# google/fedjax

Hardware: AMD Instinct MI355X
Metric: device-resident aggregated client-delta GB/s, K clients × P fp32 params (higher is better)
Workload: dtype f32; 1 GPU; configs[2]: mean aggregator, 1024 clients x 4 M-param (4,194,304) fp32 deltas; clients=1024, params=4194304, clients_per_gpu=1024, parallelism=client-sharded x1, buckets=1, nontemporal=True, variant=0, fused_l2_norms=False, fused_server_step=none

## Files before the change

fedjax_amd/csrc/fjhost.cpp:

```cpp

#include <Python.h>
#include <structmember.h>

#include <ATen/ATen.h>
#include <c10/hip/HIPFunctions.h>
#include <c10/hip/HIPStream.h>
#include <torch/csrc/autograd/python_variable.h>

#include <algorithm>
#include <chrono>
#include <cmath>
#include <cstdlib>
#include <cstdint>
#include <cstring>
#include <deque>
#include <functional>
#include <unordered_map>
#include <vector>

#include "fjagg.h"
#include "fjtree.h"

namespace {

// ... 2476 lines not shown
    std::vector<int64_t> pp(L, 0), st(3 * L, 0);
    PyObject* side[4] = {params, mt, vt, mo};
    for (int i = 0; i < 4; ++i) {
      if (side[i] == Py_None) {
        if (i == 0) Py_RETURN_NONE;
        continue;
      }
      w.out = i == 0 ? pp.data() : st.data() + (i - 1) * L;
      w.leaf = 0;
      const int r = walk(spec, side[i], w);
      if (r < 0) return nullptr;
      if (r > 0 || w.leaf != static_cast<size_t>(L)) Py_RETURN_NONE;
    }
    std::vector<int64_t> ptrs(static_cast<size_t>(K * L));
    for (int64_t l = 0; l < L; ++l) ptrs[l] = reinterpret_cast<int64_t>(row0[l].data_ptr());
    for (Py_ssize_t k = 1; k < K; ++k) {
      w.out = ptrs.data() + k * L;
      w.leaf = 0;
      const int r = walk(spec, trees[k], w);
      if (r < 0) return nullptr;
      if (r > 0 || w.leaf != static_cast<size_t>(L)) Py_RETURN_NONE;
    }
    std::vector<uint8_t> elem(L, 0);
    bool any_elem = false;
    for (int64_t l = 0; l < L; ++l) {
      int64_t bits = pp[l] | st[l] | st[L + l] | st[2 * L + l];
      for (Py_ssize_t k = 0; k < K; ++k) bits |= ptrs[k * L + l];
      elem[l] = (bits & 15) != 0;
      any_elem = any_elem || elem[l];
    }
    auto plan = reinterpret_cast<PlanFn>(plan_addr);
    const uint8_t* mask = any_elem ? elem.data() : nullptr;
    const int64_t nblk = plan(kF32, 0, leaf_n.data(), mask, static_cast<int>(L), nullptr, 0);
    if (nblk < 1) Py_RETURN_NONE;
    const int64_t nw = (K + 1) / 2, n = K * L + 2 * L + 2 * nblk + nw + 3 * L;
    if (upload_refused_in_capture(reinterpret_cast<unsigned long long>(
                                      c10::hip::getCurrentHIPStream(static_cast<c10::DeviceIndex>(dev)).stream()),
                                  "the server step's pytree fold"))
      return nullptr;
    at::Tensor img = at::empty({n}, at::TensorOptions().dtype(at::kLong).pinned_memory(true));
    int64_t* p = img.data_ptr<int64_t>();
    std::memcpy(p, ptrs.data(), sizeof(int64_t) * K * L);
    std::memcpy(p + K * L, pp.data(), sizeof(int64_t) * L);
    std::memcpy(p + K * L + L, leaf_n.data(), sizeof(int64_t) * L);
    if (plan(kF32, 0, leaf_n.data(), mask, static_cast<int>(L), p + K * L + 2 * L, nblk) != nblk) Py_RETURN_NONE;
    int64_t* wp = p + K * L + 2 * L + 2 * nblk;
    wp[nw - 1] = 0;
    std::memcpy(wp, wf.data(), 4 * K);
    std::memcpy(wp + nw, st.data(), sizeof(int64_t) * 3 * L);
    at::Tensor dimg = img.to(at::Device(at::kCUDA, static_cast<c10::DeviceIndex>(dev)), true);
    const int64_t* dp = dimg.data_ptr<int64_t>();
    const double job_bytes = 4.0 * static_cast<double>(total) * static_cast<double>(K);
    const int flags = job_bytes >= nt_min ? kNontemporal : 0;
    const float scale = static_cast<float>(W > 0.0 ? 1.0 / W : 0.0);
    const unsigned long long stream =
        reinterpret_cast<unsigned long long>(c10::hip::getCurrentHIPStream(static_cast<c10::DeviceIndex>(dev)).stream());
    const int rc = reinterpret_cast<UpdFn>(upd_addr)(kF32, dp, static_cast<int>(L), K, nblk,
                                                      reinterpret_cast<const float*>(dp + K * L + 2 * L + 2 * nblk),
                                                      scale, reinterpret_cast<const void*>(desc_addr),
                                                      dp + K * L + 2 * L + 2 * nblk + nw, flags,
                                                      reinterpret_cast<void*>(stream));
    return PyLong_FromLong(rc);
  } catch (const std::exception& e) {
    PyErr_SetString(PyExc_RuntimeError, e.what());
    return nullptr;
  }
}


struct WTObject {
  PyObject_HEAD
  PyObject* tree;
  PyObject* weight;
  PyObject* cap;
  PyObject* value;
};

struct ChainObject {
  PyObject_HEAD
  PyObject* tip;
  PyObject* buf;
  PyObject* budget;
  PyObject* views;
};

struct PSObject {
  PyObject_HEAD
  PyObject* root;
  PyObject* parent;
  PyObject* cap;
  PyObject* weight;
  PyObject* value;
  PyObject* chain;
  PyObject* ticket;
  PyObject* ref;
  PyObject* bcap;
  long long n, bytes, idx, tok;
  PyObject* weakreflist;
};

#define FJ_OBJ_MEMBER(T, f) {const_cast<char*>("_" #f), T_OBJECT, offsetof(T, f), 0, nullptr}
#define FJ_LL_MEMBER(T, f) {const_cast<char*>("_" #f), T_LONGLONG, offsetof(T, f), 0, nullptr}

PyMemberDef kWTMembers[] = {FJ_OBJ_MEMBER(WTObject, tree), FJ_OBJ_MEMBER(WTObject, weight),
                            FJ_OBJ_MEMBER(WTObject, cap), FJ_OBJ_MEMBER(WTObject, value), {nullptr}};
PyMemberDef kChainMembers[] = {{const_cast<char*>("tip"), T_OBJECT, offsetof(ChainObject, tip), 0, nullptr},
                               {const_cast<char*>("buf"), T_OBJECT, offsetof(ChainObject, buf), 0, nullptr},
                               {const_cast<char*>("budget"), T_OBJECT, offsetof(ChainObject, budget), 0, nullptr},
                               {const_cast<char*>("views"), T_OBJECT, offsetof(ChainObject, views), 0, nullptr},
                               {nullptr}};
PyMemberDef kPSMembers[] = {FJ_OBJ_MEMBER(PSObject, root),   FJ_OBJ_MEMBER(PSObject, parent),
                            FJ_OBJ_MEMBER(PSObject, cap),    FJ_OBJ_MEMBER(PSObject, weight),
                            FJ_OBJ_MEMBER(PSObject, value),  FJ_OBJ_MEMBER(PSObject, chain),
                            FJ_OBJ_MEMBER(PSObject, ticket), FJ_OBJ_MEMBER(PSObject, ref),
                            FJ_OBJ_MEMBER(PSObject, bcap),   FJ_LL_MEMBER(PSObject, n),
                            FJ_LL_MEMBER(PSObject, bytes),   FJ_LL_MEMBER(PSObject, idx),
                            FJ_LL_MEMBER(PSObject, tok),
                            {const_cast<char*>("__weaklistoffset__"), T_PYSSIZET, offsetof(PSObject, weakreflist),
                             READONLY, nullptr},
                            {nullptr}};

int wt_traverse(PyObject* o, visitproc visit, void* arg) {
  auto* x = reinterpret_cast<WTObject*>(o);
  Py_VISIT(Py_TYPE(o));
  Py_VISIT(x->tree);
  Py_VISIT(x->weight);
  Py_VISIT(x->cap);
  Py_VISIT(x->value);
  return 0;
}
int wt_clear(PyObject* o) {
  auto* x = reinterpret_cast<WTObject*>(o);
  Py_CLEAR(x->tree);
  Py_CLEAR(x->weight);
  Py_CLEAR(x->cap);
  Py_CLEAR(x->value);
  return 0;
}
void wt_dealloc(PyObject* o) {
  PyTypeObject* tp = Py_TYPE(o);
  PyObject_GC_UnTrack(o);
  wt_clear(o);
  tp->tp_free(o);
  Py_DECREF(tp);
}

int chain_traverse(PyObject* o, visitproc visit, void* arg) {
  auto* x = reinterpret_cast<ChainObject*>(o);
  Py_VISIT(Py_TYPE(o));
  Py_VISIT(x->tip);
  Py_VISIT(x->buf);
  Py_VISIT(x->budget);
  Py_VISIT(x->views);
  return 0;
}
int chain_clear(PyObject* o) {
  auto* x = reinterpret_cast<ChainObject*>(o);
  Py_CLEAR(x->tip);
  Py_CLEAR(x->buf);
  Py_CLEAR(x->budget);
  Py_CLEAR(x->views);
  return 0;
}
void chain_dealloc(PyObject* o) {
  PyTypeObject* tp = Py_TYPE(o);
  PyObject_GC_UnTrack(o);
  chain_clear(o);
  tp->tp_free(o);
  Py_DECREF(tp);
}

int ps_traverse(PyObject* o, visitproc visit, void* arg) {
  auto* x = reinterpret_cast<PSObject*>(o);
  Py_VISIT(Py_TYPE(o));
  Py_VISIT(x->root);
  Py_VISIT(x->parent);
  Py_VISIT(x->cap);
  Py_VISIT(x->weight);
  Py_VISIT(x->value);
  Py_VISIT(x->chain);
  Py_VISIT(x->ticket);
  Py_VISIT(x->ref);
  Py_VISIT(x->bcap);
  return 0;
}
int ps_clear(PyObject* o) {
  auto* x = reinterpret_cast<PSObject*>(o);
  Py_CLEAR(x->root);
  Py_CLEAR(x->parent);
  Py_CLEAR(x->cap);
  Py_CLEAR(x->weight);
  Py_CLEAR(x->value);
  Py_CLEAR(x->chain);
  Py_CLEAR(x->ticket);
  Py_CLEAR(x->ref);
  Py_CLEAR(x->bcap);
  return 0;
}
void ps_dealloc(PyObject* o) {
  PyTypeObject* tp = Py_TYPE(o);
  PyObject_GC_UnTrack(o);
  if (reinterpret_cast<PSObject*>(o)->weakreflist) PyObject_ClearWeakRefs(o);
  ps_clear(o);
  tp->tp_free(o);
  Py_DECREF(tp);
}

PyType_Slot kWTSlots[] = {{Py_tp_dealloc, reinterpret_cast<void*>(wt_dealloc)},
                          {Py_tp_traverse, reinterpret_cast<void*>(wt_traverse)},
                          {Py_tp_clear, reinterpret_cast<void*>(wt_clear)},
                          {Py_tp_members, kWTMembers},
                          {Py_tp_new, reinterpret_cast<void*>(PyType_GenericNew)},
                          {Py_tp_doc, const_cast<char*>("fields of tree_util.WeightedTree")},
                          {0, nullptr}};
PyType_Slot kChainSlots[] = {{Py_tp_dealloc, reinterpret_cast<void*>(chain_dealloc)},
                             {Py_tp_traverse, reinterpret_cast<void*>(chain_traverse)},
                             {Py_tp_clear, reinterpret_cast<void*>(chain_clear)},
                             {Py_tp_members, kChainMembers},
                             {Py_tp_new, reinterpret_cast<void*>(PyType_GenericNew)},
                             {Py_tp_doc, const_cast<char*>("fields of tree_util._Chain")},
                             {0, nullptr}};
PyType_Slot kPSSlots[] = {{Py_tp_dealloc, reinterpret_cast<void*>(ps_dealloc)},
                          {Py_tp_traverse, reinterpret_cast<void*>(ps_traverse)},
                          {Py_tp_clear, reinterpret_cast<void*>(ps_clear)},
                          {Py_tp_members, kPSMembers},
                          {Py_tp_new, reinterpret_cast<void*>(PyType_GenericNew)},
                          {Py_tp_doc, const_cast<char*>("fields of tree_util.PendingSum")},
                          {0, nullptr}};
constexpr unsigned kBaseFlags = Py_TPFLAGS_DEFAULT | Py_TPFLAGS_BASETYPE | Py_TPFLAGS_HAVE_GC;
PyType_Spec kWTSpec = {"_fjhost.WeightedBase", sizeof(WTObject), 0, kBaseFlags, kWTSlots};
PyType_Spec kChainSpec = {"_fjhost.ChainBase", sizeof(ChainObject), 0, kBaseFlags, kChainSlots};
PyType_Spec kPSSpec = {"_fjhost.PendingBase", sizeof(PSObject), 0, kBaseFlags, kPSSlots};

struct FastState {
  PyTypeObject* ticket = nullptr;
  PyTypeObject* norm_view = nullptr;
  PyObject* py_l2[2] = {nullptr, nullptr};
  PyObject* py_fold_ticket = nullptr;
  PyTypeObject* wt = nullptr;
  PyTypeObject* ps = nullptr;
  PyTypeObject* chain = nullptr;
  PyObject* py_tree_weight = nullptr;
  PyObject* py_tree_add = nullptr;
  bool defer = true;
  long long max_clients = 4095, flush_bytes = 256LL << 20, flush_clients = 64;
  PyObject* last = nullptr;
  PyObject* pool_buf = nullptr;
  PyObject* pool_views = nullptr;
  PyObject* pool_all = nullptr;
  std::vector<std::pair<PyObject*, PyObject*>> retired;
  std::vector<unsigned long long> retired_stream;
  unsigned long long pool_stream = 0;
  PyObject* d_view_ticket = nullptr;
  PyObject* d_ticket_node = nullptr;
  long long pool_want = 0;
  double refill_us = 0.0;
  long long pool_reuses = 0, pool_builds = 0;
};
FastState g_fast;

PyObject* fast_install(PyObject*, PyObject* args) {
  PyObject *wt, *ps, *ch, *ftw, *fta;
  if (!PyArg_ParseTuple(args, "O!O!O!OO", &PyType_Type, &wt, &PyType_Type, &ps, &PyType_Type, &ch, &ftw, &fta))
    return nullptr;
  if (!PyCallable_Check(ftw) || !PyCallable_Check(fta)) {
    PyErr_SetString(PyExc_TypeError, "fast_install: fallbacks must be callable");
    return nullptr;
  }
  Py_INCREF(wt), Py_INCREF(ps), Py_INCREF(ch), Py_INCREF(ftw), Py_INCREF(fta);
  Py_XSETREF(g_fast.wt, reinterpret_cast<PyTypeObject*>(wt));
  Py_XSETREF(g_fast.ps, reinterpret_cast<PyTypeObject*>(ps));
  Py_XSETREF(g_fast.chain, reinterpret_cast<PyTypeObject*>(ch));
  Py_XSETREF(g_fast.py_tree_weight, ftw);
  Py_XSETREF(g_fast.py_tree_add, fta);
  Py_RETURN_NONE;
}

PyObject* fast_config(PyObject*, PyObject* args) {
  int en;
  long long mc, fb, fc;
  if (!PyArg_ParseTuple(args, "pLLL", &en, &mc, &fb, &fc)) return nullptr;
  g_fast.defer = en != 0;
  g_fast.max_clients = mc;
  g_fast.flush_bytes = fb;
  g_fast.flush_clients = fc;
  Py_RETURN_NONE;
}

PyObject* set_last(PyObject*, PyObject* node) {
  PyObject* wr = PyWeakref_NewRef(node, nullptr);
  if (!wr) return nullptr;
  Py_XSETREF(g_fast.last, wr);
  Py_RETURN_NONE;
}
PyObject* last(PyObject*, PyObject*) {
  PyObject* o = g_fast.last ? PyWeakref_GetObject(g_fast.last) : Py_None;
  Py_INCREF(o);
  return o;
}

inline int deferrable_weight(PyObject* w) {
  if (PyFloat_CheckExact(w)) return 1;
  if (!PyLong_CheckExact(w)) return 0;
  int of = 0;
  const long long v = PyLong_AsLongLongAndOverflow(w, &of);
  if (v == -1 && PyErr_Occurred()) return -1;
  return (!of && v > -(1LL << 53) && v < (1LL << 53)) ? 1 : 0;
}

PyObject* fast_tree_weight(PyObject*, PyObject* const* args, Py_ssize_t nargs, PyObject* kwnames) {
  if (!g_fast.wt || !g_fast.py_tree_weight) {
    PyErr_SetString(PyExc_RuntimeError, "fedjax_amd.tree_util is not installed (fast_install)");
    return nullptr;
  }
  if (nargs == 2 && kwnames == nullptr) {
    const int ok = deferrable_weight(args[1]);
    if (ok < 0) return nullptr;
    if (ok) {
      PyObject* cap = capture_impl(args[0], -1);
      if (!cap) return nullptr;
      if (cap != Py_None) {
        auto* o = reinterpret_cast<WTObject*>(g_fast.wt->tp_alloc(g_fast.wt, 0));
        if (!o) {
          Py_DECREF(cap);
          return nullptr;
        }
        Py_INCREF(args[0]);
        o->tree = args[0];
        Py_INCREF(args[1]);
        o->weight = args[1];
        o->cap = cap;
        return reinterpret_cast<PyObject*>(o);
      }
      Py_DECREF(cap);
    }
  }
  return PyObject_Vectorcall(g_fast.py_tree_weight, args, nargs, kwnames);
}

inline bool flush_due(const PSObject* p) { return p->bytes >= g_fast.flush_bytes && p->n >= g_fast.flush_clients; }

PyObject* fast_tree_add(PyObject*, PyObject* const* args, Py_ssize_t nargs, PyObject* kwnames) {
  if (!g_fast.ps || !g_fast.py_tree_add) {
    PyErr_SetString(PyExc_RuntimeError, "fedjax_amd.tree_util is not installed (fast_install)");
    return nullptr;
  }
  if (nargs == 2 && kwnames == nullptr && g_fast.defer && Py_TYPE(args[1]) == g_fast.wt &&
      Py_TYPE(args[0]) == g_fast.ps) {
    auto* r = reinterpret_cast<WTObject*>(args[1]);
    auto* p = reinterpret_cast<PSObject*>(args[0]);
    auto* ch = reinterpret_cast<ChainObject*>(p->chain);
    if (r->tree && r->tree != Py_None && r->cap && PyTuple_CheckExact(r->cap) && PyTuple_GET_SIZE(r->cap) >= 4 &&
        (!p->value || p->value == Py_None) && p->tok >= 0 && ch && Py_TYPE(ch) == g_fast.chain &&
        ch->tip == args[0] && ch->budget && PyLong_CheckExact(ch->budget)) {
      const long long tok = PyLong_AsLongLong(PyTuple_GET_ITEM(r->cap, 3));
      const long long nb = PyLong_AsLongLong(PyTuple_GET_ITEM(r->cap, 2));
      const long long budget = PyLong_AsLongLong(ch->budget);
      if (PyErr_Occurred()) return nullptr;
      if (tok == p->tok && p->n + 1 <= g_fast.max_clients && p->bytes + nb <= budget && !flush_due(p)) {
        auto* q = reinterpret_cast<PSObject*>(g_fast.ps->tp_alloc(g_fast.ps, 0));
        if (!q) return nullptr;
        Py_INCREF(p);
        q->parent = args[0];
        Py_INCREF(r->cap);
        q->cap = r->cap;
        Py_INCREF(r->weight);
        q->weight = r->weight;
        Py_INCREF(ch);
        q->chain = reinterpret_cast<PyObject*>(ch);
        Py_XINCREF(p->ref);
        q->ref = p->ref;
        q->n = p->n + 1;
        q->bytes = p->bytes + nb;
        q->idx = p->idx + 1;
        q->tok = p->tok;
        Py_INCREF(q);
        Py_XSETREF(ch->tip, reinterpret_cast<PyObject*>(q));
        PyObject* wr = PyWeakref_NewRef(reinterpret_cast<PyObject*>(q), nullptr);
        if (!wr) {
          Py_DECREF(q);
          return nullptr;
        }
        Py_XSETREF(g_fast.last, wr);
        return reinterpret_cast<PyObject*>(q);
      }
    }
  }
  return PyObject_Vectorcall(g_fast.py_tree_add, args, nargs, kwnames);
}


PyObject* fast_install_norms(PyObject*, PyObject* args) {
  PyObject *tk, *nv, *f0, *f1, *ft = Py_None;
  if (!PyArg_ParseTuple(args, "O!O!OO|O", &PyType_Type, &tk, &PyType_Type, &nv, &f0, &f1, &ft)) return nullptr;
  Py_INCREF(tk), Py_INCREF(nv), Py_INCREF(f0), Py_INCREF(f1), Py_INCREF(ft);
  Py_XSETREF(g_fast.ticket, reinterpret_cast<PyTypeObject*>(tk));
  Py_XSETREF(g_fast.norm_view, reinterpret_cast<PyTypeObject*>(nv));
  Py_XSETREF(g_fast.py_l2[0], f0);
  Py_XSETREF(g_fast.py_l2[1], f1);
  Py_XSETREF(g_fast.py_fold_ticket, ft);
  PyObject* dv = PyObject_GetAttrString(nv, "_ticket");
  PyObject* dn = dv ? PyObject_GetAttrString(tk, "node") : nullptr;
  if (!dv || !dn || !Py_TYPE(dv)->tp_descr_set || !Py_TYPE(dn)->tp_descr_set || !Py_TYPE(dv)->tp_descr_get) {
    Py_XDECREF(dv), Py_XDECREF(dn);
    PyErr_Clear();
    PyErr_SetString(PyExc_TypeError, "fast_install_norms: _NormView._ticket and _Ticket.node must be __slots__");
    return nullptr;
  }
  Py_XSETREF(g_fast.d_view_ticket, dv);
  Py_XSETREF(g_fast.d_ticket_node, dn);
  Py_RETURN_NONE;
}

inline int slot_set(PyObject* descr, PyObject* obj, PyObject* v) { return Py_TYPE(descr)->tp_descr_set(descr, obj, v); }

PyObject* solo_stale_error() {
  PyErr_SetString(PyExc_RuntimeError,
                  "a client delta passed to tree_l2_norm / tree_l2_squared was modified (a leaf updated in place) "
                  "before its lazy norm was computed; the reference takes the norm of the value at that call. Add "
                  "copies, or call fedjax_amd.tree_util.set_lazy_norms(False)");
  return nullptr;
}

PyObject* solo_config(PyObject*, PyObject* args) {
  int on;
  long long mp, bb;
  unsigned long long rf, wf, pf;
  PyObject* pb;
  if (!PyArg_ParseTuple(args, "pLLKKKO", &on, &mp, &bb, &rf, &wf, &pf, &pb)) return nullptr;
  g_solo.on = on != 0;
  g_solo.max_pending = std::max<long long>(1, std::min<long long>(mp, 1LL << 20));
  g_solo.budget = std::max<long long>(0, bb);
  if (rf) g_solo.rows_fn = rf;
  if (wf) g_solo.l2ws_fn = wf;
  if (pf) g_solo.plan_fn = pf;
  if (pb != Py_None) {
    Py_INCREF(pb);
    Py_XSETREF(g_solo.py_budget, pb);
  }
  Py_RETURN_NONE;
}

// ... 747 lines not shown
    links.push_back(p);
    if (!p->parent || p->parent == Py_None) {
      base = p->root;
      break;
    }
    if (Py_TYPE(p->parent) != g_fast.ps) Py_RETURN_NONE;
    p = reinterpret_cast<PSObject*>(p->parent);
  }
  if (links.empty() || !base) Py_RETURN_NONE;
  std::reverse(links.begin(), links.end());
  PyObject* bcap = links[0]->bcap;
  if (!bcap || bcap == Py_None) Py_RETURN_NONE;
  const Py_ssize_t K = static_cast<Py_ssize_t>(links.size()) + 1;
  thread_local std::vector<PyObject*> caps, weights;
  caps.resize(K);
  weights.resize(K);
  static PyObject* one = PyLong_FromLong(1);
  caps[0] = bcap;
  weights[0] = one;
  for (Py_ssize_t j = 1; j < K; ++j) {
    caps[j] = links[j - 1]->cap;
    weights[j] = links[j - 1]->weight;
    if (!caps[j] || !weights[j]) Py_RETURN_NONE;
  }
  static PyObject* node_name = PyUnicode_InternFromString("node");
  thread_local std::vector<size_t> waiting;
  waiting.clear();
  for (size_t j = 0; j < links.size(); ++j) {
    PyObject* tk = links[j]->ticket;
    if (!tk || tk == Py_None) continue;
    PyObject* tn = (Py_TYPE(tk) == g_fast.ticket && g_fast.d_ticket_node)
                       ? Py_TYPE(g_fast.d_ticket_node)->tp_descr_get(g_fast.d_ticket_node, tk, nullptr)
                       : PyObject_GetAttr(tk, node_name);
    if (!tn) return nullptr;
    const bool w = tn != Py_None;
    Py_DECREF(tn);
    if (w) waiting.push_back(j);
  }
  try {
    L2Rows rows{};
    bool use_rows = false;
    c10::DeviceIndex rows_dev = -1;
    if (!waiting.empty() && rows_addr) {
      PyObject* ch0 = links[0]->chain;
      bool one = ch0 && Py_TYPE(ch0) == g_fast.chain;
      for (size_t j = 1; one && j < links.size(); ++j)
        one = links[j]->chain == ch0 && links[j]->idx == links[0]->idx + static_cast<long long>(j);
      PyObject* buf = one ? reinterpret_cast<ChainObject*>(ch0)->buf : nullptr;
      if (buf && THPVariable_Check(buf)) {
        const at::Tensor& b = THPVariable_Unpack(buf);
        const int64_t i0 = links[0]->idx, n = static_cast<int64_t>(links.size());
        PyObject* bt0 = PyTuple_Check(bcap) && PyTuple_GET_SIZE(bcap) > 0 ? PyTuple_GET_ITEM(bcap, 0) : nullptr;
        const int fold_dev = bt0 && PyTuple_Check(bt0) && PyTuple_GET_SIZE(bt0) > 0 &&
                                     THPVariable_Check(PyTuple_GET_ITEM(bt0, 0))
                                 ? THPVariable_Unpack(PyTuple_GET_ITEM(bt0, 0)).get_device()
                                 : -2;
        if (b.dim() == 2 && b.size(0) == 2 && b.is_contiguous() && b.scalar_type() == at::kFloat && b.is_cuda() &&
            b.get_device() == fold_dev && i0 >= 0 && i0 + n <= b.size(1)) {
          float* row0 = b.data_ptr<float>() + i0;
          rows = L2Rows{reinterpret_cast<WsumL2RowsFn>(rows_addr), row0, row0 + b.size(1), 1};
          use_rows = true;
          rows_dev = b.get_device();
        }
      }
    }
    at::Tensor l2;
    PyObject* l2obj = Py_None;
    if (!waiting.empty() && !use_rows) {
      PyObject* t0 = PyTuple_Check(bcap) && PyTuple_GET_SIZE(bcap) > 0 ? PyTuple_GET_ITEM(bcap, 0) : nullptr;
      if (!t0 || !PyTuple_Check(t0) || PyTuple_GET_SIZE(t0) < 1 || !THPVariable_Check(PyTuple_GET_ITEM(t0, 0)))
        Py_RETURN_NONE;
      l2 = at::empty({K}, THPVariable_Unpack(PyTuple_GET_ITEM(t0, 0)).options().dtype(at::kFloat));
      l2obj = THPVariable_Wrap(l2);
      if (!l2obj) return nullptr;
    }
    Py_INCREF(base);
    PyObject* got = fold_caps_impl(base, caps.data(), weights.data(), K, scale, has_scale != 0, nt_min, plan_addr,
                                   wsum_addr, l2_addr, l2ws_addr, l2obj, use_rows ? &rows : nullptr);
    if (got && PyTuple_Check(got)) {
      const double now = now_s();
      const auto* tip = reinterpret_cast<PSObject*>(node);
      const double bytes = static_cast<double>(tip->bytes) * (1.0 + 1.0 / std::max<long long>(1, tip->n));
      g_mean.busy_until = std::max(now, g_mean.busy_until) + bytes / g_mean.peak;
    }
    Py_DECREF(base);
    if (l2obj != Py_None) Py_DECREF(l2obj);
    if (!got || waiting.empty() || !PyTuple_Check(got) || PyLong_AsLong(PyTuple_GET_ITEM(got, 0)) != 0) return got;
    typedef int (*FillFn)(const float*, float*, float*, int64_t, void*);
    auto fill = reinterpret_cast<FillFn>(fill_addr);
    for (size_t j = use_rows ? links.size() : 0; j < links.size();) {
      PyObject* ch = links[j]->chain;
      const size_t j0 = j;
      while (j < links.size() && links[j]->chain == ch &&
             links[j]->idx == links[j0]->idx + static_cast<long long>(j - j0))
        ++j;
      PyObject* buf = ch && Py_TYPE(ch) == g_fast.chain ? reinterpret_cast<ChainObject*>(ch)->buf : nullptr;
      if (buf && THPVariable_Check(buf)) {
        const at::Tensor& b = THPVariable_Unpack(buf);
        const int64_t i0 = links[j0]->idx, n = std::min<int64_t>(static_cast<int64_t>(j - j0), b.size(1) - i0);
        if (n <= 0) continue;
        if (fill && b.is_contiguous() && b.scalar_type() == at::kFloat && b.is_cuda() &&
            b.get_device() == l2.get_device()) {
          float* row0 = b.data_ptr<float>() + i0;
          const hipStream_t s = c10::hip::getCurrentHIPStream(l2.get_device()).stream();
          const int rc = fill(l2.data_ptr<float>() + 1 + j0, row0, row0 + b.size(1), n, s);
          if (rc != 0) {
            Py_DECREF(got);
            PyErr_Format(PyExc_RuntimeError, "fjtree_norms_fill failed (%d)", rc);
            return nullptr;
          }
          continue;
        }
        const at::Tensor src = l2.narrow(0, 1 + static_cast<int64_t>(j0), n);
        b.select(0, 0).narrow(0, i0, n).copy_(src);
        at::Tensor dst = b.select(0, 1).narrow(0, i0, n);
        at::sqrt_out(dst, src);
      }
    }
    for (size_t j : waiting) {
      PyObject* tk = links[j]->ticket;
      if ((Py_TYPE(tk) == g_fast.ticket && g_fast.d_ticket_node ? slot_set(g_fast.d_ticket_node, tk, Py_None)
                                                                 : PyObject_SetAttr(tk, node_name, Py_None)) != 0) {
        Py_DECREF(got);
        return nullptr;
      }
      Py_CLEAR(links[j]->ticket);
    }
    if (has_scale) {
      auto* ch = reinterpret_cast<ChainObject*>(links.back()->chain);
      if (ch && Py_TYPE(ch) == g_fast.chain && ch->tip == node) {
        Py_CLEAR(ch->buf);
        Py_CLEAR(ch->views);
      }
      if (refill_pool(use_rows ? rows_dev : l2.get_device()) != 0) {
        Py_DECREF(got);
        return nullptr;
      }
    }
    return got;
  } catch (const std::exception& e) {
    PyErr_SetString(PyExc_RuntimeError, e.what());
    return nullptr;
  }
}

PyObject* image_paths(PyObject*, PyObject*) {
  return Py_BuildValue("{s:L,s:L}", "kernel_args", g_image_karg, "uploaded", g_image_upload);
}

PyObject* host_timers(PyObject*, PyObject*) {
  static const char* names[kTPhases] = {"spec",  "checks", "outputs", "plan",           "image",
                                        "upload", "launch", "wrap",    "first_launch_at"};
  PyObject* d = PyDict_New();
  if (!d) return nullptr;
  for (int i = 0; i < kTPhases; ++i) {
    PyObject* v = PyFloat_FromDouble(g_timer_calls ? g_timers[i] / g_timer_calls : 0.0);
    PyDict_SetItemString(d, names[i], v);
    Py_DECREF(v);
    g_timers[i] = 0.0;
  }
  PyObject* c = PyLong_FromLongLong(g_timer_calls);
  PyDict_SetItemString(d, "calls", c);
  Py_DECREF(c);
  g_timer_calls = 0;
  return d;
}

PyMethodDef kMethods[] = {
    {"host_timers", host_timers, METH_NOARGS, "mean per-call microseconds of fold_table's phases (resets)"},
    {"image_paths", image_paths, METH_NOARGS, "fold_table launches with the image in kernel arguments / uploaded"},
    {"gather_rows", gather_rows, METH_VARARGS, "pointer table of K client pytrees (see fjhost.cpp)"},
    {"leaf_versions", leaf_versions, METH_VARARGS, "torch in-place version counters of K pytrees' leaves"},
    {"fold_weights", fold_weights, METH_VARARGS, "f32/i32 weights and W of Python-number weights"},
    {"capture", capture, METH_VARARGS, "leaves + version sum of a tree for a lazy tree_weight"},
    {"capture_probe", capture_probe, METH_VARARGS, "ns per call of capture's parts (profiling)"},
    {"solo_probe", solo_probe, METH_VARARGS, "ns per call of the lazy norm capture's parts (profiling)"},
    {"matches", matches, METH_VARARGS, "tree holds exactly the captured leaves, unmodified"},
    {"compatible", compatible, METH_VARARGS, "tree_add(a, b) is the fast case (structure, float32 leaves)"},
    {"append_check", append_check, METH_VARARGS, "deferred tree_add: structure + capture check in one walk"},
    {"norm_view", norm_view, METH_VARARGS, "0-d view of buf[row, index] as a tensor subclass"},
    {"table_from_caps", table_from_caps, METH_VARARGS, "pointer table of captured leaves, version check"},
    {"fold_caps", fold_caps, METH_VARARGS, "a deferred running sum's fold from its captures, one call"},
    {"leaf_fold", leaf_fold, METH_VARARGS, "fjtree_fold_leaves over 1-2 operand trees (see fjhost.cpp)"},
    {"fold_table", fold_table, METH_VARARGS, "plan image + output leaves + fjagg_wsum_ptrs launch (see fjhost.cpp)"},
    {"mean_pairs", mean_pairs, METH_VARARGS, "tree_mean of (pytree, weight) pairs in one native call (see fjhost.cpp)"},
    {"server_pairs", server_pairs, METH_VARARGS, "fused_tree_mean_update in one native call (see fjhost.cpp)"},
    {"zeros_like", zeros_like, METH_O, "tree_zeros_like of a float32 device pytree: one allocation, own leaves"},
    {"mean_config", mean_config, METH_VARARGS, "configuration of the builtin tree_mean (tree_util._native_mean)"},
    {"tree_mean", reinterpret_cast<PyCFunction>(reinterpret_cast<void*>(fast_tree_mean)), METH_FASTCALL | METH_KEYWORDS,
     "tree_mean(pytrees_and_weights)\n--\n\nReturns (weighted) mean of input trees and weights "
     "(fedjax/core/tree_util.py:76-96).\n\nA resident list / tuple of (float32 device pytree, Python-number weight) "
     "pairs is folded by one native call\n(the pytree kernel, pipelined with the walk on an idle GPU); every other "
     "input is\nfedjax_amd.tree_util._tree_mean_py's (one-shot iterables stream in chunks).\n\nThe result's "
     "float32 leaves are slices of one allocation (each its own tensor and\nversion counter): one live leaf keeps "
     "all of them allocated, and torch.save of one\nleaf writes every leaf's bytes (clone a leaf to keep it alone)."},
    {"mean_triples", mean_triples, METH_O, "tree_mean over (client_id, params, weight) triples (aggregator.py:61-75)"},
    {"pipeline_fracs", pipeline_fracs, METH_O, "chunk ends (fractions of K) of tree_mean's fold-bound pipeline"},
    {"busy_until", busy_until, METH_VARARGS, "the shared estimate of when this process's folds finish ([set])"},
    {"fold_chain", fold_chain, METH_VARARGS, "a PendingSum's deferred fold, its links walked natively"},
    {"flush_views", flush_views, METH_O, "fold the chains lazy norm views in an object still wait on"},
    {"fast_install_norms", fast_install_norms, METH_VARARGS, "register tree_util's lazy norm classes and fallbacks"},
    {"drop_pool", drop_pool, METH_NOARGS, "forget the lazy-norm pool"},
    {"solo_config", solo_config, METH_VARARGS, "standalone lazy norms: switch, limits, library entry points"},
    {"solo_resolve", solo_resolve_py, METH_O, "compute pending standalone lazy norms now (None: all)"},
    {"solo_info", solo_info, METH_NOARGS, "standalone lazy norms: pending, fused, computed alone, stale"},
    {"solo_norm", solo_norm_py, METH_VARARGS, "the standalone lazy norm view of a tree, or None"},
    {"solo_times", solo_times, METH_NOARGS, "host us the means spent releasing, compacting, refilling (resets)"},
    {"pool_info", pool_info, METH_NOARGS, "(pool views ready, norms asked for since the last refill)"},
    {"tree_l2_squared", reinterpret_cast<PyCFunction>(reinterpret_cast<void*>(fast_tree_l2_squared)),
     METH_FASTCALL | METH_KEYWORDS,
     "tree_l2_squared(pytree)\n--\n\nReturns squared l2 norm of tree (fedjax/core/tree_util.py:105-108), a 0-d "
     "float32 tensor.\n\nThe delta a deferred running sum just took gets a lazy view its fold fills; anything "
     "else is\nfedjax_amd.tree_util._tree_l2_squared_py."},
    {"tree_l2_norm", reinterpret_cast<PyCFunction>(reinterpret_cast<void*>(fast_tree_l2_norm)),
     METH_FASTCALL | METH_KEYWORDS,
     "tree_l2_norm(pytree)\n--\n\nReturns l2 norm of tree (fedjax/core/tree_util.py:111-114), a 0-d float32 "
     "tensor.\n\nThe delta a deferred running sum just took gets a lazy view its fold fills; anything else "
     "is\nfedjax_amd.tree_util._tree_l2_norm_py."},
    {"fast_install", fast_install, METH_VARARGS, "register tree_util's lazy classes and Python fallbacks"},
    {"fast_config", fast_config, METH_VARARGS, "deferred-sum settings (tree_util.set_deferred_sums)"},
    {"set_last", set_last, METH_O, "remember the most recent PendingSum link (weakly)"},
    {"last", last, METH_NOARGS, "the most recent PendingSum link, or None"},
    {"tree_weight", reinterpret_cast<PyCFunction>(reinterpret_cast<void*>(fast_tree_weight)),
     METH_FASTCALL | METH_KEYWORDS,
     "tree_weight(pytree, weight)\n--\n\nWeights tree leaves by weight (fedjax/core/tree_util.py:29-32).\n\n"
     "Float32 device pytrees (<= 64 leaves) with a Python-number weight give a WeightedTree\n"
     "(deferred, fused into the tree_add that consumes it); anything else is computed now\n"
     "by the pytree kernel (fedjax_amd.tree_util._tree_weight_py)."},
    {"tree_add", reinterpret_cast<PyCFunction>(reinterpret_cast<void*>(fast_tree_add)), METH_FASTCALL | METH_KEYWORDS,
     "tree_add(left, right)\n--\n\nAdds two trees together (fedjax/core/tree_util.py:47-50).\n\n"
     "The running sum s = tree_add(s, tree_weight(x, n)) appends to a deferred PendingSum\n"
     "(one launch folds the round); every other case is fedjax_amd.tree_util._tree_add_py."},
    {nullptr, nullptr, 0, nullptr},
};

PyModuleDef kModule = {PyModuleDef_HEAD_INIT, "_fjhost", "native host side of the pytree aggregation path",
                       -1, kMethods};

}

#ifndef FJHOST_TORCH_STAMP
#define FJHOST_TORCH_STAMP "unstamped"
#endif

PyMODINIT_FUNC PyInit__fjhost(void) {
  PyObject* m = PyModule_Create(&kModule);
  if (!m) return nullptr;
  if (PyModule_AddStringConstant(m, "TORCH_STAMP", FJHOST_TORCH_STAMP) != 0) {
    Py_DECREF(m);
    return nullptr;
  }
  const std::pair<const char*, PyType_Spec*> types[] = {
      {"WeightedBase", &kWTSpec}, {"ChainBase", &kChainSpec}, {"PendingBase", &kPSSpec}, {"SoloNorm", &kSoloSpec}};
  for (const auto& t : types) {
    PyObject* tp = PyType_FromSpec(t.second);
    if (tp && t.second == &kSoloSpec) {
      Py_INCREF(tp);
      g_solo.type = reinterpret_cast<PyTypeObject*>(tp);
    }
    if (!tp || PyModule_AddObject(m, t.first, tp) != 0) {
      Py_XDECREF(tp);
      Py_DECREF(m);
      return nullptr;
    }
  }
  return m;
}
```

fedjax_amd/tree_util.py:

```python

from __future__ import annotations

import copy
import ctypes
import numbers
import os
import time
import weakref
from typing import Any, Iterable, List, Optional, Sequence, Tuple

import numpy as np
import torch

from fedjax_amd import _lib, kernels, pytree
from fedjax_amd.typing import PyTree

__all__ = [
    "tree_weight", "tree_inverse_weight", "tree_zeros_like", "tree_add", "tree_sum",
    "tree_mean", "tree_size", "tree_l2_squared", "tree_l2_norm", "tree_clip_by_global_norm",
    "tree_l2_norms", "tree_mean_with_l2_norms", "WeightedTree", "PendingSum", "set_deferred_sums",
    "set_lazy_norms", "set_bf16_semantics", "bf16_semantics",
]

NONTEMPORAL_MIN_BYTES = 256 << 20
# ... 444 lines not shown
_NORM_COMBINE = os.environ.get("FJTREE_NORM_COMBINE", "handoff")


def set_norm_combine(mode: str) -> None:
    global _NORM_COMBINE
    if mode not in ("handoff", "ordered"):
        raise ValueError("norm combine is 'handoff' or 'ordered'")
    _NORM_COMBINE = mode


def _leaf_fold(trees, weights, caps, scale=None, norm_operand=-1, no_out=False):
    fold, ws = _TREE_ADDRS or _tree_addrs()
    flags = ((_lib.SCALE if scale is not None else 0) | (_lib.TREE_NORM if norm_operand >= 0 else 0)
             | (_lib.TREE_NO_OUT if no_out else 0)
             | (_lib.TREE_ORDERED if norm_operand >= 0 and _NORM_COMBINE == "ordered" else 0))
    got = _lib.host().leaf_fold(trees, weights, caps, 1.0 if scale is None else float(scale), flags,
                                max(norm_operand, 0), -1, 0, fold, ws)
    if got is None:
        return None
    rc, out, sq, l2 = got
    if rc == _STALE:
        raise RuntimeError("a pytree passed to tree_weight was modified (a leaf replaced or updated in "
                           "place) before its weighted value was used; the reference computes "
                           "tree_weight eagerly")
    _lib.check(rc, "fjtree_fold_leaves")
    return out, sq, l2


_HOST = _lib.host()


class WeightedTree(_HOST.WeightedBase):

    __slots__ = ()

    def __init__(self, tree, weight, cap):
        self._tree, self._weight, self._cap, self._value = tree, weight, cap, None

    def materialize(self) -> PyTree:
        if self._value is None:
            from fedjax_amd import memory
            with memory.producing(self._cap[0][0].device if memory.default_enabled() else None):
                got = _leaf_fold([self._tree], [self._weight], [self._cap])
            if got is None:
                raise RuntimeError("the pytree passed to tree_weight changed structure before use")
            self._value = got[0]
            self._tree = self._cap = None
        return self._value

    def __getitem__(self, key):
        return self.materialize()[key]

    def __iter__(self):
        return iter(self.materialize())

    def __len__(self):
        return len(self.materialize())

    def __contains__(self, key):
        return key in self.materialize()

    def __getattr__(self, name):
        if name.startswith("__"):
            raise AttributeError(name)
        return getattr(self.materialize(), name)

    def __repr__(self):
        return f"WeightedTree({self.materialize()!r})"

    def __reduce_ex__(self, proto):
        return copy.copy, (self.materialize(),)

    def __deepcopy__(self, memo):
        return copy.deepcopy(self.materialize(), memo)

    def __copy__(self):
        return copy.copy(self.materialize())


pytree.register_lazy_type(WeightedTree, WeightedTree.materialize)
_F32_EXACT_INT = 1 << 53

_DEFER = {"enabled": True, "budget_bytes": None, "max_clients": 4095,
          "flush_bytes": 256 << 20, "flush_clients": 64}
_AUTO_BUDGET = {}


def set_deferred_sums(enabled: bool = True, *, budget_bytes: Optional[int] = None,
                      max_clients: Optional[int] = None, flush_bytes: Optional[int] = None,
                      flush_clients: Optional[int] = None) -> None:
    _DEFER["enabled"] = bool(enabled)
    if budget_bytes is not None:
        _DEFER["budget_bytes"] = int(budget_bytes) if int(budget_bytes) > 0 else None
    if max_clients is not None:
        _DEFER["max_clients"] = min(4095, max(1, int(max_clients)))
    if flush_bytes is not None:
        _DEFER["flush_bytes"] = max(0, int(flush_bytes))
    if flush_clients is not None:
        _DEFER["flush_clients"] = max(1, int(flush_clients))
    _HOST.fast_config(_DEFER["enabled"], _DEFER["max_clients"], _DEFER["flush_bytes"], _DEFER["flush_clients"])
    _HOST.drop_pool()


_LAZY = {"enabled": os.environ.get("FJAGG_LAZY_NORMS", "1") != "0", "budget_bytes": None, "max_pending": 16383}


def set_lazy_norms(enabled: bool = True, *, budget_bytes: Optional[int] = None,
                   max_pending: Optional[int] = None) -> None:
    _LAZY["enabled"] = bool(enabled)
    if budget_bytes is not None:
        _LAZY["budget_bytes"] = int(budget_bytes) if int(budget_bytes) > 0 else None
    if max_pending is not None:
        _LAZY["max_pending"] = max(1, min(1 << 20, int(max_pending)))
    _solo_config()


def _solo_budget(dev: int) -> int:
    return _defer_budget(torch.device("cuda", dev))


def _solo_config() -> None:
    if _ENTRY_ADDRS is None:
        _HOST.solo_config(_LAZY["enabled"], _LAZY["max_pending"], _LAZY["budget_bytes"] or 0, 0, 0, 0, _solo_budget)
        return
    _HOST.solo_config(_LAZY["enabled"], _LAZY["max_pending"], _LAZY["budget_bytes"] or 0, _ROWS_ADDR,
                      _ENTRY_ADDRS[3], _ENTRY_ADDRS[0], _solo_budget)


def _defer_budget(device: torch.device) -> int:
    b = _DEFER["budget_bytes"]
    if b is not None:
        return b
    idx = device.index if device.index is not None else torch.cuda.current_device()
    got = _AUTO_BUDGET.get(idx)
    if got is None:
        free, _ = torch.cuda.mem_get_info(idx)
        got = _AUTO_BUDGET[idx] = int(min(4 << 30, max(64 << 20, free // 8)))
    return got


class _Chain(_HOST.ChainBase):

    __slots__ = ()

    def __init__(self):
        self.tip, self.buf, self.budget = None, None, None


class _Ticket:

    __slots__ = ("node",)

    def __init__(self, node):
        self.node = node


class _NormView(torch.Tensor):

    __slots__ = ("_ticket",)

    @classmethod
    def __torch_function__(cls, func, types, args=(), kwargs=None):
        _HOST.flush_views(args)
        if kwargs:
            _HOST.flush_views(kwargs)
        with torch._C.DisableTorchFunctionSubclass():
            return func(*args, **(kwargs or {}))

    def __format__(self, spec):
        _HOST.flush_views(self)
        with torch._C.DisableTorchFunctionSubclass():
            return self.item().__format__(spec) if self.dim() == 0 else torch.Tensor.__format__(self, spec)

    def _value(self) -> torch.Tensor:
        _HOST.flush_views(self)
        with torch._C.DisableTorchFunctionSubclass():
            return self.detach().clone()

    def __reduce_ex__(self, proto):
        return torch.Tensor.__reduce_ex__(self._value(), proto)

    def __deepcopy__(self, memo):
        return self._value()
# ... 150 lines not shown
        raise RuntimeError("the running sum passed to tree_add was modified (a leaf replaced or updated in "
                           "place) before the pending sum was used; the reference adds its value at tree_add. "
                           "Call fedjax_amd.tree_util.set_deferred_sums(False) for loops that do this")
    raise RuntimeError(f"client {bad - 1} of a pending tree_add sum was modified (a leaf updated in place) "
                       "after its tree_weight / tree_add; the reference sums each delta's value at that "
                       "call. Add copies, or call fedjax_amd.tree_util.set_deferred_sums(False)")


def _fill_norms(links, waiting, l2sq):
    j = 0
    while j < len(links):
        ch, j0 = links[j]._chain, j
        while j < len(links) and links[j]._chain is ch and links[j]._idx == links[j0]._idx + (j - j0):
            j += 1
        if ch.buf is not None:
            i0 = links[j0]._idx
            n = min(j - j0, ch.buf.shape[1] - i0)
            if n > 0:
                src, cols = l2sq[1 + j0:1 + j0 + n], ch.buf.shape[1]
                _lib.check(_lib.load().fjtree_norms_fill(
                    src.data_ptr(), ch.buf.data_ptr() + 4 * i0, ch.buf.data_ptr() + 4 * (cols + i0), n,
                    torch.cuda.current_stream(src.device).cuda_stream), "fjtree_norms_fill")
    for n in waiting:
        n._ticket.node = None
        n._ticket = None


def _lazy_norm(pytree_, row: int):
    node = _HOST.last()
    if node is None or node._value is not None or node._cap is None:
        return None
    host = _HOST
    if not host.matches(pytree_, node._cap[0], node._cap[1]):
        return None
    ch = node._chain
    if ch.buf is None:
        ch.buf = torch.empty((2, _DEFER["max_clients"] + 1), dtype=torch.float32, device=node._cap[0][0].device)
    if node._idx >= ch.buf.shape[1]:
        return None
    if node._ticket is None:
        node._ticket = _Ticket(node)
    v = host.norm_view(ch.buf, row, node._idx, _NormView)
    v._ticket = node._ticket
    return v


def _defer(sum_side, item, item_weight, item_cap):
    host = _HOST
    if type(sum_side) is PendingSum:
        parent, root = sum_side, None
        live = sum_side._value is None
        ref = sum_side._ref if live else sum_side._value
    else:
        ref, parent, root, live = sum_side, None, sum_side, False
    bcap = None
    if live:
        tok = parent._tok
    else:
        bcap = host.capture(ref, -1)
        tok = bcap[3] if bcap is not None else -1
    if item_cap is not None and tok >= 0 and item_cap[3] == tok:
        cap = item_cap
    else:
        cap = host.append_check(ref, item, item_cap)
        if cap is None:
            return None
        if type(cap) is int:
            raise RuntimeError("a pytree passed to tree_weight was modified (a leaf replaced or updated in "
                               "place) before its weighted value was used; the reference computes "
                               "tree_weight eagerly")
    if live:
        budget = parent._chain.budget
        if budget is None:
            budget = parent._chain.budget = _defer_budget(cap[0][0].device)
        if parent._n + 1 > _DEFER["max_clients"] or parent._bytes + cap[2] > budget or _flush_due(parent):
            parent.materialize()
            bcap = host.capture(parent._value, -1)
    node = PendingSum(root, parent, cap, item_weight, ref, bcap, tok)
    host.set_last(node)
    return node


def _flush_due(p: "PendingSum") -> bool:
    return p._bytes >= _DEFER["flush_bytes"] and p._n >= _DEFER["flush_clients"]


def _tree_weight_py(pytree_: PyTree, weight: float) -> PyTree:
    tw = type(weight)
    w = weight if (tw is float or tw is int) else _host_weight(weight)
    if (type(w) is float or (type(w) is int and -_F32_EXACT_INT < w < _F32_EXACT_INT)):
        cap = _HOST.capture(pytree_, -1)
        if cap is not None:
            return WeightedTree(pytree_, w, cap)
    return _fold_trees([pytree_], [w])


def _eager(t):
    return t.materialize() if type(t) is WeightedTree or type(t) is PendingSum else t


def tree_inverse_weight(pytree_: PyTree, weight: float) -> PyTree:
    inv = _inverse(weight if type(weight) is float or type(weight) is int else _host_weight(weight))
    if type(pytree_) is PendingSum and pytree_._value is None:
        return _fold_pending(pytree_, inv)
    pytree_ = _eager(pytree_)
    if type(inv) is float:
        got = _leaf_fold([pytree_], [inv], [None])
        if got is not None:
            return got[0]
    return _fold_trees([pytree_], [inv])


def tree_zeros_like(pytree_: PyTree) -> PyTree:
    got = _HOST.zeros_like(pytree_)
    if got is not None:
        return got
    leaves, td = pytree.flatten(pytree_)
    device = _find_device(leaves)
    out = []
    for x in leaves:
        t = _to_tensor(x)
        dt = _CANONICAL.get(t.dtype)
        if dt is None:
            raise TypeError(f"leaf dtype {t.dtype} is not supported")
        out.append(torch.zeros(t.shape, dtype=dt, device=device))
    return pytree.unflatten(td, out)


def _tree_add_py(left: PyTree, right: PyTree) -> PyTree:
    tl, tr = type(left) is WeightedTree, type(right) is WeightedTree
    if tr and not tl and right._tree is not None and _DEFER["enabled"]:
        got = _defer(left, right._tree, right._weight, right._cap)
        if got is not None:
            return got
    pl, pr = type(left) is PendingSum, type(right) is PendingSum
    if _DEFER["enabled"] and (tl != tr or pl != pr) and not (pl and pr):
        if tr and right._tree is not None and not tl:
            got = _defer(left, right._tree, right._weight, right._cap)
        elif tl and left._tree is not None and not tr:
            got = _defer(right, left._tree, left._weight, left._cap)
        elif pl and not tr:
            got = _defer(left, right, 1, None)
        elif pr and not tl:
            got = _defer(right, left, 1, None)
        else:
            got = None
        if got is not None:
            return got
    left, right = (left.materialize() if pl else left), (right.materialize() if pr else right)
    if tl or tr:
        ops = [left._tree if tl else left, right._tree if tr else right]
        if ops[0] is None or ops[1] is None:
            return _fold_trees([_eager(left), _eager(right)], [1, 1])
        ws = [left._weight if tl else 1, right._weight if tr else 1]
        caps = [left._cap if tl else None, right._cap if tr else None]
        norm_op = 1 if tr else 0
    else:
        ops, ws, caps, norm_op = [left, right], [1, 1], [None, None], -1
    got = _leaf_fold(ops, ws, caps, norm_operand=norm_op)
    if got is not None:
        out, sq, l2 = got
        if norm_op >= 0:
            _NORMS.appendleft((caps[norm_op], sq, l2))
        return out
    return _fold_trees([_eager(left), _eager(right)], [1, 1])


_HOST.fast_install(WeightedTree, PendingSum, _Chain, _tree_weight_py, _tree_add_py)
_HOST.fast_config(_DEFER["enabled"], _DEFER["max_clients"], _DEFER["flush_bytes"], _DEFER["flush_clients"])
DEFERRED_SUM_DEFAULTS = {"max_clients": _DEFER["max_clients"], "flush_bytes": _DEFER["flush_bytes"],
                         "flush_clients": _DEFER["flush_clients"], "budget_bytes": 0}
tree_weight = _HOST.tree_weight
tree_add = _HOST.tree_add


def tree_sum(pytrees: Iterable[PyTree]) -> PyTree:
    trees = list(pytrees)
    if not trees:
        return None
    return _fold_trees(trees, [1] * len(trees))


def _collect_pairs(pairs):
    if type(pairs) is not list:
        pairs = list(pairs)
    trees = [tree for tree, _ in pairs]
    weights = [weight for _, weight in pairs]
    packed = _pack_weights(weights) if trees else None
    if packed is not None:
        return trees, packed, packed.total
    sum_weight = 0.0
    for i, w in enumerate(weights):
        w = weights[i] = _host_weight(w)
        sum_weight += w
    return trees, weights, sum_weight


_PIPELINE_FRAC = float(os.environ.get("FJAGG_PIPELINE_FRAC", "0.2"))
_PIPELINE_CHUNK = int(os.environ.get("FJAGG_PIPELINE_CHUNK", "512"))
_PIPELINE_MIN_BYTES = 64 << 20
_WALK_NS_PER_LEAF = 35.0
_PEAK_BYTES_PER_S = 8.0e12
class _BusyUntil:

    __slots__ = ()

    def __getitem__(self, i):
        return _HOST.busy_until()

    def __setitem__(self, i, t):
        _HOST.busy_until(float(t))


_BUSY_UNTIL = _BusyUntil()


_NATIVE_MEAN = os.environ.get("FJAGG_NATIVE_MEAN", "1") != "0"


def _native_mean(pairs, with_l2: bool = False):
    if _ENTRY_ADDRS is None:
        _native_fold_addrs()
    now = time.perf_counter()
    extra = (_ENTRY_ADDRS[2], _ENTRY_ADDRS[3]) if with_l2 else ()
    got = _lib.host().mean_pairs(pairs, _PIPELINE_FRAC > 0.0 and now >= _BUSY_UNTIL[0], _PIPELINE_FRAC,
                                 _PIPELINE_CHUNK, _CHUNK_WALK_US, _WALK_NS_PER_LEAF, _PIPELINE_MIN_BYTES,
                                 _NARROW_MAX_BYTES, float(NONTEMPORAL_MIN_BYTES), _ENTRY_ADDRS[0], _ENTRY_ADDRS[1],
                                 *extra)
    if got is None:
        return None
    rc, tree, job_bytes, l2sq = got
    _BUSY_UNTIL[0] = max(now, _BUSY_UNTIL[0]) + job_bytes / _PEAK_BYTES_PER_S
    _lib.check(rc, "fjagg_wsum_l2_ptrs" if with_l2 else "fjagg_wsum_ptrs")
    return (tree, l2sq) if with_l2 else tree


def _stream_idle(stream: torch.cuda.Stream) -> bool:
    return stream.query()


_CHUNK_WALK_US = 60.0


def _pipeline_bounds(K: int, n: int, L: int) -> List[int]:
    walk_ns, fold_ns = _WALK_NS_PER_LEAF * L, 4.0 * n / _PEAK_BYTES_PER_S * 1e9
    if walk_ns > fold_ns and _PIPELINE_CHUNK > 0:
        c = max(_PIPELINE_CHUNK, int(np.ceil(_CHUNK_WALK_US * 1e3 / walk_ns)))
        if K > c:
            return list(range(c, K, c)) + [K]
    return [min(K - 1, max(1, int(K * _PIPELINE_FRAC))), K]


def _tree_mean_pipelined(trees: List[PyTree], packed: "_Weights", W, first) -> Optional[PyTree]:
    leaves0, td = first
# ... 279 lines not shown
```

Measured before the change: 7080 GB/s.

## Hold back early deferred-sum flushes while the stream is still busy folding

Adds a host-side estimate of when each device stream's pending chain folds finish, updated whenever a fold is launched. When a deferred sum reaches its flush threshold, the flush is postponed for a number of further clients if the stream is still estimated busy. The aim is bigger fold batches and less launch overhead, without letting the GPU go idle. It adds per-tree_add stream lookups and a heuristic whose timing depends on an assumed peak bandwidth, and it is on by default.

Measured after the change: 7080 GB/s. No clear change (-0.0%).

```diff
diff --git a/fedjax_amd/csrc/fjhost.cpp b/fedjax_amd/csrc/fjhost.cpp
--- a/fedjax_amd/csrc/fjhost.cpp
+++ b/fedjax_amd/csrc/fjhost.cpp
@@ -2582,6 +2582,8 @@
   PyObject* buf;
   PyObject* budget;
   PyObject* views;
+  long long ask_idx, ask_next;
+  int ask_flush;
 };
 
 struct PSObject {
@@ -2744,6 +2746,7 @@
   PyObject* py_tree_add = nullptr;
   bool defer = true;
   long long max_clients = 4095, flush_bytes = 256LL << 20, flush_clients = 64;
+  bool hold = true;
   PyObject* last = nullptr;
   PyObject* pool_buf = nullptr;
   PyObject* pool_views = nullptr;
@@ -2777,9 +2780,10 @@
 }
 
 PyObject* fast_config(PyObject*, PyObject* args) {
-  int en;
+  int en, hold = g_fast.hold ? 1 : 0;
   long long mc, fb, fc;
-  if (!PyArg_ParseTuple(args, "pLLL", &en, &mc, &fb, &fc)) return nullptr;
+  if (!PyArg_ParseTuple(args, "pLLL|p", &en, &mc, &fb, &fc, &hold)) return nullptr;
+  g_fast.hold = hold != 0;
   g_fast.defer = en != 0;
   g_fast.max_clients = mc;
   g_fast.flush_bytes = fb;
@@ -2838,7 +2842,114 @@
   return PyObject_Vectorcall(g_fast.py_tree_weight, args, nargs, kwnames);
 }
 
-inline bool flush_due(const PSObject* p) { return p->bytes >= g_fast.flush_bytes && p->n >= g_fast.flush_clients; }
+constexpr double kFlushMargin = 40e-6;
+struct FlushState {
+  long long early = 0, held = 0, queries = 0;
+  int force = 0;
+  std::unordered_map<uint64_t, double> busy_until;
+};
+FlushState g_flush;
+
+inline uint64_t flush_stream_key(int dev, unsigned long long stream) {
+  return static_cast<uint64_t>(stream) ^ (static_cast<uint64_t>(dev) << 56);
+}
+
+bool flush_stream_of(const PSObject* p, int* dev, unsigned long long* stream) {
+  PyObject* t0 = p->cap && PyTuple_Check(p->cap) && PyTuple_GET_SIZE(p->cap) > 0 ? PyTuple_GET_ITEM(p->cap, 0) : nullptr;
+  if (!t0 || !PyTuple_Check(t0) || PyTuple_GET_SIZE(t0) < 1 || !THPVariable_Check(PyTuple_GET_ITEM(t0, 0)))
+    return false;
+  const at::Tensor& x = THPVariable_Unpack(PyTuple_GET_ITEM(t0, 0));
+  if (!x.is_cuda()) return false;
+  try {
+    *dev = x.get_device();
+    *stream = reinterpret_cast<unsigned long long>(
+        c10::hip::getCurrentHIPStream(static_cast<c10::DeviceIndex>(*dev)).stream());
+    return true;
+  } catch (const std::exception&) {
+    return false;
+  }
+}
+
+void flush_note_fold(const PSObject* tip, double bytes, double now) {
+  int dev;
+  unsigned long long stream;
+  if (!flush_stream_of(tip, &dev, &stream) || stream_capturing(stream)) return;
+  if (g_flush.busy_until.size() >= 64) g_flush.busy_until.clear();
+  double& t = g_flush.busy_until[flush_stream_key(dev, stream)];
+  t = std::max(now, t) + bytes / g_mean.peak;
+}
+
+int flush_stream_busy(const PSObject* p) {
+  int dev;
+  unsigned long long stream;
+  if (!flush_stream_of(p, &dev, &stream)) return -1;
+  bool busy = g_flush.force == 1;
+  if (!g_flush.force) {
+    const auto it = g_flush.busy_until.find(flush_stream_key(dev, stream));
+    busy = it != g_flush.busy_until.end() && it->second - now_s() > kFlushMargin;
+  }
+  if (busy && stream_capturing(stream)) return -1;
+  ++g_flush.queries;
+  return busy ? 1 : 0;
+}
+
+bool flush_due(const PSObject* p, ChainObject* ch) {
+  if (p->bytes < g_fast.flush_bytes || p->n < g_fast.flush_clients) return false;
+  if (ch && ch->ask_idx == p->idx + 1) return ch->ask_flush != 0;
+  bool flush = true;
+  if (g_fast.hold && ch) {
+    if (ch->ask_idx > 0 && !ch->ask_flush && p->idx < ch->ask_next) {
+      flush = false;
+    } else {
+      const int busy = flush_stream_busy(p);
+      if (busy == 1) {
+        flush = false;
+        ch->ask_next = p->idx + std::max<long long>(1, g_fast.flush_clients / 4);
+      }
+    }
+  }
+  if (ch) ch->ask_idx = p->idx + 1, ch->ask_flush = flush ? 1 : 0;
+  ++(flush ? g_flush.early : g_flush.held);
+  return flush;
+}
+
+PyObject* flush_due_py(PyObject*, PyObject* node) {
+  if (!g_fast.ps || !PyObject_TypeCheck(node, g_fast.ps)) {
+    PyErr_SetString(PyExc_TypeError, "flush_due: a PendingSum link");
+    return nullptr;
+  }
+  auto* p = reinterpret_cast<PSObject*>(node);
+  auto* ch = p->chain && g_fast.chain && Py_TYPE(p->chain) == g_fast.chain ? reinterpret_cast<ChainObject*>(p->chain)
+                                                                           : nullptr;
+  return PyBool_FromLong(flush_due(p, ch) ? 1 : 0);
+}
+
+PyObject* flush_busy_until(PyObject*, PyObject* args) {
+  int dev;
+  unsigned long long stream;
+  double t = -1.0;
+  if (!PyArg_ParseTuple(args, "iK|d", &dev, &stream, &t)) return nullptr;
+  const uint64_t key = flush_stream_key(dev, stream);
+  if (t >= 0.0) g_flush.busy_until[key] = t;
+  const auto it = g_flush.busy_until.find(key);
+  return PyFloat_FromDouble(it != g_flush.busy_until.end() ? it->second : 0.0);
+}
+
+PyObject* flush_info(PyObject*, PyObject*) {
+  return Py_BuildValue("{s:L,s:L,s:L,s:i,s:i}", "early", g_flush.early, "held", g_flush.held, "queries",
+                       g_flush.queries, "hold", g_fast.hold ? 1 : 0, "force", g_flush.force);
+}
+
+PyObject* flush_hold_force(PyObject*, PyObject* arg) {
+  const long v = PyLong_AsLong(arg);
+  if (v == -1 && PyErr_Occurred()) return nullptr;
+  if (v < 0 || v > 2) {
+    PyErr_SetString(PyExc_ValueError, "flush_hold_force: 0 (the estimate), 1 (busy) or 2 (drained)");
+    return nullptr;
+  }
+  g_flush.force = static_cast<int>(v);
+  Py_RETURN_NONE;
+}
 
 PyObject* fast_tree_add(PyObject*, PyObject* const* args, Py_ssize_t nargs, PyObject* kwnames) {
   if (!g_fast.ps || !g_fast.py_tree_add) {
@@ -2857,7 +2968,7 @@
       const long long nb = PyLong_AsLongLong(PyTuple_GET_ITEM(r->cap, 2));
       const long long budget = PyLong_AsLongLong(ch->budget);
       if (PyErr_Occurred()) return nullptr;
-      if (tok == p->tok && p->n + 1 <= g_fast.max_clients && p->bytes + nb <= budget && !flush_due(p)) {
+      if (tok == p->tok && p->n + 1 <= g_fast.max_clients && p->bytes + nb <= budget && !flush_due(p, ch)) {
         auto* q = reinterpret_cast<PSObject*>(g_fast.ps->tp_alloc(g_fast.ps, 0));
         if (!q) return nullptr;
         Py_INCREF(p);
@@ -3771,6 +3882,7 @@
       const auto* tip = reinterpret_cast<PSObject*>(node);
       const double bytes = static_cast<double>(tip->bytes) * (1.0 + 1.0 / std::max<long long>(1, tip->n));
       g_mean.busy_until = std::max(now, g_mean.busy_until) + bytes / g_mean.peak;
+      flush_note_fold(tip, bytes, now);
     }
     Py_DECREF(base);
     if (l2obj != Py_None) Py_DECREF(l2obj);
@@ -3908,6 +4020,10 @@
      "is\nfedjax_amd.tree_util._tree_l2_norm_py."},
     {"fast_install", fast_install, METH_VARARGS, "register tree_util's lazy classes and Python fallbacks"},
     {"fast_config", fast_config, METH_VARARGS, "deferred-sum settings (tree_util.set_deferred_sums)"},
+    {"flush_due", flush_due_py, METH_O, "fold a PendingSum's pending run before the next link (early flush)?"},
+    {"flush_info", flush_info, METH_NOARGS, "early flushes taken / held back, answers asked for, switches"},
+    {"flush_busy_until", flush_busy_until, METH_VARARGS, "a stream's estimate of when its chain folds finish ([set])"},
+    {"flush_hold_force", flush_hold_force, METH_O, "force the early flush's stream answer (0 real, 1 busy, 2 drained)"},
     {"set_last", set_last, METH_O, "remember the most recent PendingSum link (weakly)"},
     {"last", last, METH_NOARGS, "the most recent PendingSum link, or None"},
     {"tree_weight", reinterpret_cast<PyCFunction>(reinterpret_cast<void*>(fast_tree_weight)),
diff --git a/fedjax_amd/tree_util.py b/fedjax_amd/tree_util.py
--- a/fedjax_amd/tree_util.py
+++ b/fedjax_amd/tree_util.py
@@ -550,13 +550,14 @@
 _F32_EXACT_INT = 1 << 53
 
 _DEFER = {"enabled": True, "budget_bytes": None, "max_clients": 4095,
-          "flush_bytes": 256 << 20, "flush_clients": 64}
+          "flush_bytes": 256 << 20, "flush_clients": 64,
+          "hold_while_busy": os.environ.get("FJAGG_FLUSH_HOLD", "1") != "0"}
 _AUTO_BUDGET = {}
 
 
 def set_deferred_sums(enabled: bool = True, *, budget_bytes: Optional[int] = None,
                       max_clients: Optional[int] = None, flush_bytes: Optional[int] = None,
-                      flush_clients: Optional[int] = None) -> None:
+                      flush_clients: Optional[int] = None, hold_while_busy: Optional[bool] = None) -> None:
     _DEFER["enabled"] = bool(enabled)
     if budget_bytes is not None:
         _DEFER["budget_bytes"] = int(budget_bytes) if int(budget_bytes) > 0 else None
@@ -566,7 +567,10 @@
         _DEFER["flush_bytes"] = max(0, int(flush_bytes))
     if flush_clients is not None:
         _DEFER["flush_clients"] = max(1, int(flush_clients))
-    _HOST.fast_config(_DEFER["enabled"], _DEFER["max_clients"], _DEFER["flush_bytes"], _DEFER["flush_clients"])
+    if hold_while_busy is not None:
+        _DEFER["hold_while_busy"] = bool(hold_while_busy)
+    _HOST.fast_config(_DEFER["enabled"], _DEFER["max_clients"], _DEFER["flush_bytes"], _DEFER["flush_clients"],
+                      _DEFER["hold_while_busy"])
     _HOST.drop_pool()
 
 
@@ -883,7 +887,7 @@
 
 
 def _flush_due(p: "PendingSum") -> bool:
-    return p._bytes >= _DEFER["flush_bytes"] and p._n >= _DEFER["flush_clients"]
+    return _HOST.flush_due(p)
 
 
 def _tree_weight_py(pytree_: PyTree, weight: float) -> PyTree:
@@ -968,9 +972,11 @@
 
 
 _HOST.fast_install(WeightedTree, PendingSum, _Chain, _tree_weight_py, _tree_add_py)
-_HOST.fast_config(_DEFER["enabled"], _DEFER["max_clients"], _DEFER["flush_bytes"], _DEFER["flush_clients"])
+_HOST.fast_config(_DEFER["enabled"], _DEFER["max_clients"], _DEFER["flush_bytes"], _DEFER["flush_clients"],
+                  _DEFER["hold_while_busy"])
 DEFERRED_SUM_DEFAULTS = {"max_clients": _DEFER["max_clients"], "flush_bytes": _DEFER["flush_bytes"],
-                         "flush_clients": _DEFER["flush_clients"], "budget_bytes": 0}
+                         "flush_clients": _DEFER["flush_clients"], "budget_bytes": 0,
+                         "hold_while_busy": _DEFER["hold_while_busy"]}
 tree_weight = _HOST.tree_weight
 tree_add = _HOST.tree_add
 
```
